# AI4Science-WestlakeU/wdno

Hardware: AMD Instinct MI355X
Metric: diffusion train steps/sec, 2D smoke U-Net (8 samples per GPU per step) (higher is better)
Workload: dtype f32

## Files before the change

### wdno_amd/csrc/conv_prep.hip

```cpp
#include "conv_tiles.h"
#include <algorithm>

template <bool RECORD>
__global__ __launch_bounds__(256) void amax_kernel(const float* __restrict__ x, int64_t n, unsigned* __restrict__ out) {
  __shared__ float red[4];
  const int64_t n4 = n >> 2;
  const float4* x4 = reinterpret_cast<const float4*>(x);
  float m = 0.f;
  const int64_t stride = (int64_t)gridDim.x * 1024;
  for (int64_t k0 = (int64_t)blockIdx.x * 1024 + threadIdx.x; k0 < n4; k0 += stride) {
    float4 v[4];
#pragma unroll
    for (int u = 0; u < 4; ++u) {
      int64_t k = k0 + u * 256;
      v[u] = k < n4 ? x4[k] : make_float4(0.f, 0.f, 0.f, 0.f);
    }
#pragma unroll
    for (int u = 0; u < 4; ++u)
      m = fmaxf(fmaxf(m, fmaxf(fabsf(v[u].x), fabsf(v[u].y))), fmaxf(fabsf(v[u].z), fabsf(v[u].w)));
  }
  if (blockIdx.x == 0)
    for (int64_t k = (n4 << 2) + threadIdx.x; k < n; k += 256) m = fmaxf(m, fabsf(x[k]));
  if (RECORD) {
    amax_record_emit(m, reinterpret_cast<float*>(out), blockIdx.x);
    return;
  }
  m = wave_max(m);
  if ((threadIdx.x & 63) == 0) red[threadIdx.x >> 6] = m;
  __syncthreads();
  if (threadIdx.x == 0) {
    m = fmaxf(fmaxf(red[0], red[1]), fmaxf(red[2], red[3]));
    atomicMax(out, __float_as_uint(m));
  }
}
void conv_amax_record_launch(const float* x, int64_t n, float* rec, hipStream_t st) {
  amax_kernel<true><<<stream_grid(n / 16 + 1, 256), 256, 0, st>>>(x, n, reinterpret_cast<unsigned*>(rec));
}
extern "C" int wdno_amax_record(const float* x, int64_t n, float* rec_zeroed, wdno_stream_t s) {
  WDNO_REQUIRE(n >= 0);
  if (n == 0) return WDNO_OK;
  amax_kernel<true><<<stream_grid(n / 16 + 1, 256), 256, 0, as_stream(s)>>>(x, n, reinterpret_cast<unsigned*>(rec_zeroed));
  return wdno_check_launch();
}
extern "C" int wdno_amax(const float* x, int64_t n, float* amax_zeroed, wdno_stream_t s) {
  WDNO_REQUIRE(n > 0);
  amax_kernel<false><<<stream_grid(n / 16 + 1, 256), 256, 0, as_stream(s)>>>(x, n, reinterpret_cast<unsigned*>(amax_zeroed));
  return wdno_check_launch();
}

__global__ __launch_bounds__(256) void split_kernel(const float* __restrict__ x, const float* __restrict__ amax,
                                                     _Float16* __restrict__ hi, _Float16* __restrict__ lo, float* __restrict__ scale_out,
                                                     int64_t rows, int C, int C8) {
  const bool lp = lo == nullptr;
  const float s = lp ? 1.0f : scale_from_amax(amax_record_read(amax));
  if (!lp && blockIdx.x == 0 && threadIdx.x == 0) scale_out[0] = s;
  const int g8 = C8 >> 3;
  const int64_t total = rows * g8;
  const int64_t stride = (int64_t)gridDim.x * 256;
  for (int64_t i = (int64_t)blockIdx.x * 256 + threadIdx.x; i < total; i += stride) {
    int64_t r = i / g8;
    int c0 = (int)(i - r * g8) * 8;
    float v[8];
    const float* xp = x + r * C + c0;
    if (c0 + 8 <= C) {
      float4 a = *reinterpret_cast<const float4*>(xp), b = *reinterpret_cast<const float4*>(xp + 4);
      v[0] = a.x; v[1] = a.y; v[2] = a.z; v[3] = a.w; v[4] = b.x; v[5] = b.y; v[6] = b.z; v[7] = b.w;
    } else {
#pragma unroll
      for (int e = 0; e < 8; ++e) v[e] = (c0 + e < C) ? xp[e] : 0.f;
    }
    if (lp) {
      typedef unsigned short us8 __attribute__((ext_vector_type(8)));
      us8 b;
#pragma unroll
      for (int e = 0; e < 8; ++e) b[e] = bf16_rne(v[e]);
      *reinterpret_cast<us8*>(hi + r * C8 + c0) = b;
      continue;
    }
    half8 h, l;
#pragma unroll
    for (int e = 0; e < 8; ++e) {
      float t = v[e] * s;
      _Float16 th = (_Float16)t;
      h[e] = th;
      l[e] = (_Float16)(t - (float)th);
    }
    *reinterpret_cast<half8*>(hi + r * C8 + c0) = h;
    *reinterpret_cast<half8*>(lo + r * C8 + c0) = l;
  }
}
extern "C" int wdno_cast_bf16(const float* x, void* out, int64_t rows, int C, int C8, wdno_stream_t s) {
  WDNO_REQUIRE(rows > 0 && C > 0 && (C & 3) == 0 && (C8 & 7) == 0 && C8 >= C && C8 < C + 16);
  int64_t total = rows * (C8 / 8);
  split_kernel<<<stream_grid(total, 256), 256, 0, as_stream(s)>>>(x, nullptr, (_Float16*)out, nullptr, nullptr, rows, C, C8);
  return wdno_check_launch();
}
extern "C" int wdno_split_f16(const float* x, const float* amax, void* hi, void* lo, float* scale_out, int64_t rows, int C, int C8,
                              wdno_stream_t s) {
  WDNO_REQUIRE(rows > 0 && C > 0 && (C & 3) == 0 && (C8 & 7) == 0 && C8 >= C && C8 < C + 16);
  int64_t total = rows * (C8 / 8);
  split_kernel<<<stream_grid(total, 256), 256, 0, as_stream(s)>>>(x, amax, (_Float16*)hi, (_Float16*)lo, scale_out, rows, C, C8);
  return wdno_check_launch();
}

__global__ __launch_bounds__(256) void split_colsum_kernel(const float* __restrict__ x, const float* __restrict__ amax,
                                                            _Float16* __restrict__ hi, _Float16* __restrict__ lo, float* __restrict__ scale_out,
                                                            double* __restrict__ part, int64_t rows, int C, int C8) {
  __shared__ float red[256][9];
  const bool lp = lo == nullptr;
  const float s = lp ? 1.0f : scale_from_amax(amax_record_read(amax));
  if (!lp && blockIdx.x == 0 && threadIdx.x == 0) scale_out[0] = s;
  const int g8 = C8 >> 3;
  const int64_t total = rows * g8;
  const int64_t stride = (int64_t)gridDim.x * 256;
  float cs[8];
#pragma unroll
  for (int e = 0; e < 8; ++e) cs[e] = 0.f;
  for (int64_t i = (int64_t)blockIdx.x * 256 + threadIdx.x; i < total; i += stride) {
    int64_t r = i / g8;
    int c0 = (int)(i - r * g8) * 8;
    float v[8];
    const float* xp = x + r * C + c0;
    if (c0 + 8 <= C) {
      float4 a = *reinterpret_cast<const float4*>(xp), b = *reinterpret_cast<const float4*>(xp + 4);
      v[0] = a.x; v[1] = a.y; v[2] = a.z; v[3] = a.w; v[4] = b.x; v[5] = b.y; v[6] = b.z; v[7] = b.w;
    } else {
#pragma unroll
      for (int e = 0; e < 8; ++e) v[e] = (c0 + e < C) ? xp[e] : 0.f;
    }
    if (lp) {
      typedef unsigned short us8 __attribute__((ext_vector_type(8)));
      us8 b;
#pragma unroll
      for (int e = 0; e < 8; ++e) { cs[e] += v[e]; b[e] = bf16_rne(v[e]); }
      *reinterpret_cast<us8*>(hi + r * C8 + c0) = b;
      continue;
    }
    half8 h, l;
#pragma unroll
    for (int e = 0; e < 8; ++e) {
      cs[e] += v[e];
      float t = v[e] * s;
      _Float16 th = (_Float16)t;
      h[e] = th;
      l[e] = (_Float16)(t - (float)th);
    }
    *reinterpret_cast<half8*>(hi + r * C8 + c0) = h;
    *reinterpret_cast<half8*>(lo + r * C8 + c0) = l;
  }
#pragma unroll
  for (int e = 0; e < 8; ++e) red[threadIdx.x][e] = cs[e];
  __syncthreads();
  for (int idx = threadIdx.x; idx < C8; idx += 256) {
    const int grp = idx >> 3, e = idx & 7;
    double acc = 0.0;
    for (int t = grp; t < 256; t += g8) acc += (double)red[t][e];
    part[(int64_t)blockIdx.x * C8 + idx] = acc;
  }
}
extern "C" size_t wdno_split_colsum_ws_bytes(int64_t rows, int C8) {
  return (size_t)stream_grid(rows * (C8 / 8), 256) * (size_t)C8 * sizeof(double);
}
extern "C" int wdno_split_f16_colsum(const float* x, const float* amax, void* hi, void* lo, float* scale_out, float* colsum_out,
                                     void* ws, size_t ws_bytes, int64_t rows, int C, int C8, wdno_stream_t s) {
  WDNO_REQUIRE(rows > 0 && C > 0 && (C & 3) == 0 && (C8 & 7) == 0 && C8 >= C && C8 < C + 16);
  const int g8 = C8 / 8;
  if (g8 > 256 || (g8 & (g8 - 1))) return WDNO_EUNSUPPORTED;
  if (ws_bytes < wdno_split_colsum_ws_bytes(rows, C8)) return WDNO_EWORKSPACE;
  const int grid = stream_grid(rows * g8, 256);
  split_colsum_kernel<<<grid, 256, 0, as_stream(s)>>>(x, amax, (_Float16*)hi, (_Float16*)lo, scale_out, (double*)ws, rows, C, C8);
  if (colsum_out)
    partial_rows_sum_kernel<double><<<cdiv(C8, 32), PRS_THREADS, 0, as_stream(s)>>>((const double*)ws, colsum_out, grid, C8);
  return wdno_check_launch();
}

extern "C" int wdno_cast_bf16_colsum(const float* x, void* out, float* colsum_out, void* ws, size_t ws_bytes, int64_t rows, int C, int C8,
                                     wdno_stream_t s) {
  WDNO_REQUIRE(rows > 0 && C > 0 && (C & 3) == 0 && (C8 & 7) == 0 && C8 >= C && C8 < C + 16);
  const int g8 = C8 / 8;
  if (g8 > 256 || (g8 & (g8 - 1))) return WDNO_EUNSUPPORTED;
  if (ws_bytes < wdno_split_colsum_ws_bytes(rows, C8)) return WDNO_EWORKSPACE;
  const int grid = stream_grid(rows * g8, 256);
  split_colsum_kernel<<<grid, 256, 0, as_stream(s)>>>(x, nullptr, (_Float16*)out, nullptr, nullptr, (double*)ws, rows, C, C8);
  if (colsum_out)
    partial_rows_sum_kernel<double><<<cdiv(C8, 32), PRS_THREADS, 0, as_stream(s)>>>((const double*)ws, colsum_out, grid, C8);
  return wdno_check_launch();
}

#define PS_LDS_FLOATS 10240
struct PackTile { int KT, CT, CTp, tiles_k, tiles_c; };
__host__ __device__ static inline PackTile pack_tile(int T, int A, int B, int mode) {
  PackTile t;
  auto need = [&](int longd, int shortd) { return (int64_t)T * (mode ? (int64_t)longd * (shortd + 1) : (int64_t)shortd * (longd + 1)); };
  int longd = 128, shortd = 8;
  while (longd > 8 && need(longd, shortd) > PS_LDS_FLOATS) longd >>= 1;
  while (shortd > 1 && need(longd, shortd) > PS_LDS_FLOATS) shortd >>= 1;
  t.KT = mode ? longd : shortd;
  t.CT = mode ? shortd : longd;
  t.CTp = t.CT + 1;
  const int kext = mode ? B : A, cext = mode ? A : B;
  t.tiles_k = (kext + t.KT - 1) / t.KT;
  t.tiles_c = (cext + t.CT - 1) / t.CT;
  return t;
}
__device__ __forceinline__ unsigned ps_magic(unsigned d) { return d > 1 ? (unsigned)((1ull << 32) / d) + 1u : 0u; }
__device__ __forceinline__ int ps_div(int n, int d, unsigned m) { return d == 1 ? n : (int)__umulhi((unsigned)n, m); }
__device__ __forceinline__ void pack_split_body(const float* __restrict__ w, const float* __restrict__ amax,
                                                _Float16* __restrict__ hi, _Float16* __restrict__ lo,
                                                float* __restrict__ scale_out, int K, int C, int kd, int kh, int kw,
                                                int A, int B, int mode_in, int block, int nblocks) {
  __shared__ float tile[PS_LDS_FLOATS + 16];
  const int frag = mode_in >= 10 ? mode_in - 9 : 0;
  const int parity = mode_in >= 2 && mode_in < 6 ? mode_in - 2 : -1;
  const int patch = mode_in >= 6 && mode_in < 10 ? mode_in - 6 : -1;
  const int mode = mode_in == 1 || patch >= 0 ? 1 : 0;
  const bool lp = lo == nullptr;
  const float s = lp ? 1.0f : scale_from_amax(amax[0]);
  if (!lp && block == 0 && threadIdx.x == 0) scale_out[0] = s;
  const int b8 = B >> 3;
  const int T = kd * kh * kw, khw = kh * kw;
  const PackTile pt = pack_tile(T, A, B, mode);
  if ((int64_t)T * pt.KT * pt.CTp > PS_LDS_FLOATS + 16) return;
  const int ntiles = pt.tiles_k * pt.tiles_c;
  const int run = pt.CT * T;
  const int bt8 = (mode ? pt.KT : pt.CT) >> 3;
  const int at = mode ? pt.CT : pt.KT;
  const unsigned m_run = ps_magic(run), m_T = ps_magic(T), m_bt8 = ps_magic(bt8), m_at = ps_magic(at), m_khw = ps_magic(khw), m_kw = ps_magic(kw);
  for (int tl = block; tl < ntiles; tl += nblocks) {
    const int tk = ps_div(tl, pt.tiles_c, ps_magic(pt.tiles_c)), tc = tl - tk * pt.tiles_c;
    const int k0 = tk * pt.KT, c0 = tc * pt.CT;
    __syncthreads();
    const int cvalid = min(pt.CT, C - c0);
    const int nload = pt.KT * run;
    for (int idx0 = threadIdx.x; idx0 < nload; idx0 += 256 * 8) {
      float v[8];
      int dst[8];
#pragma unroll
      for (int u = 0; u < 8; ++u) {
        const int idx = min(idx0 + 256 * u, nload - 1);
        const int kk = ps_div(idx, run, m_run), r = idx - kk * run;
        const int cl = ps_div(r, T, m_T), tap = r - cl * T;
        const bool ok = k0 + kk < K && cl < cvalid;
        const int64_t off = !ok ? 0 : patch >= 0 ? (((int64_t)(k0 + kk) * C + c0 + cl) * 4 + patch) : parity < 0 ? ((int64_t)(k0 + kk) * C + c0) * T + r
                            : ((int64_t)(c0 + cl) * K + (k0 + kk)) * 16 + (3 - (parity >> 1) - 2 * (tap >> 1)) * 4 + (3 - (parity & 1) - 2 * (tap & 1));
        v[u] = w[off];
        if (!ok) v[u] = 0.f;
        dst[u] = idx0 + 256 * u < nload ? (tap * pt.KT + kk) * pt.CTp + cl : -1;
      }
#pragma unroll
      for (int u = 0; u < 8; ++u)
        if (dst[u] >= 0) tile[dst[u]] = v[u];
    }
    __syncthreads();
    const int nitems = T * at * bt8;
    for (int idx = threadIdx.x; idx < nitems; idx += 256) {
      int q = ps_div(idx, bt8, m_bt8);
      const int g = idx - q * bt8;
      const int tap = ps_div(q, at, m_at), al = q - tap * at;
      const int dz = ps_div(tap, khw, m_khw), rr = tap - dz * khw;
      const int dy = ps_div(rr, kw, m_kw), dx = rr - dy * kw;
      const int ts = mode ? T - 1 - tap : tap;
      const int a = (mode ? c0 : k0) + al;
      const int bg = ((mode ? k0 : c0) >> 3) + g;
      if (a >= A || bg >= b8) continue;
      const float* src = mode ? tile + (ts * pt.KT + g * 8) * pt.CTp + al : tile + (ts * pt.KT + al) * pt.CTp + g * 8;
      const int step = mode ? pt.CTp : 1;
      half8 h, l;
      typedef unsigned short us8 __attribute__((ext_vector_type(8)));
      us8 bq;
#pragma unroll
      for (int e = 0; e < 8; ++e) {
        const float v = src[e * step];
        const float tv = v * s;
        const _Float16 th = (_Float16)tv;
        h[e] = th;
        l[e] = (_Float16)(tv - (float)th);
        bq[e] = bf16_rne(v);
      }
      int64_t i = ((((int64_t)dz * kh + dy) * A + a) * kw + dx) * b8 + bg;
      if (frag) {
        const int li = a & 31, t = bg >> 2, hh2 = (bg >> 1) & 1, s2 = bg & 1;
        if (frag == 1) { const int ti = a >> 7, hd = (a >> 5) & 3; i = ((((hd * 3 + ti) * (B >> 5) + t) * 2 + s2) * 64 + hh2 * 32 + li); }
        else { const int q4 = A >> 2, wv = a / q4, mt = (a - wv * q4) >> 5; i = ((((wv * (A >> 7) + mt) * 4 + t) * 2 + s2) * 64 + hh2 * 32 + li); }
      }
      if (lp) { *reinterpret_cast<us8*>(hi + i * 8) = bq; continue; }
      *reinterpret_cast<half8*>(hi + i * 8) = h;
      *reinterpret_cast<half8*>(lo + i * 8) = l;
    }
  }
}
__global__ __launch_bounds__(256) void pack_split_weight_kernel(const float* __restrict__ w, const float* __restrict__ amax,
                                                                 _Float16* __restrict__ hi, _Float16* __restrict__ lo,
                                                                 float* __restrict__ scale_out, int K, int C, int kd, int kh, int kw,
                                                                 int A, int B, int mode) {
  pack_split_body(w, amax, hi, lo, scale_out, K, C, kd, kh, kw, A, B, mode, (int)blockIdx.x, (int)gridDim.x);
}
__global__ __launch_bounds__(256) void amax_multi_kernel(const wdno_amax_item* __restrict__ tab) {
  __shared__ float red[4];
  const wdno_amax_item it = tab[blockIdx.y];
  const float* x = (const float*)it.x;
  const int64_t n = it.n;
  float m = 0.f;
  int64_t head = (int64_t)(((16 - (reinterpret_cast<uintptr_t>(x) & 15)) & 15) >> 2);
  if (head > n) head = n;
  const int64_t n4 = (n - head) >> 2, tail0 = head + 4 * n4;
  if (blockIdx.x == 0) {
    if ((int64_t)threadIdx.x < head) m = fabsf(x[threadIdx.x]);
    if (tail0 + (int64_t)threadIdx.x < n) m = fmaxf(m, fabsf(x[tail0 + threadIdx.x]));
  }
  const float4* x4 = reinterpret_cast<const float4*>(x + head);
  const int64_t stride = (int64_t)gridDim.x * 256;
  int64_t k = (int64_t)blockIdx.x * 256 + threadIdx.x;
  for (; k + 3 * stride < n4; k += 4 * stride) {
    const float4 a = x4[k], b = x4[k + stride], c = x4[k + 2 * stride], d = x4[k + 3 * stride];
    m = amax4(amax4(m, a), b);
    m = amax4(amax4(m, c), d);
  }
  for (; k < n4; k += stride) m = amax4(m, x4[k]);
  m = wave_max(m);
  if ((threadIdx.x & 63) == 0) red[threadIdx.x >> 6] = m;
  __syncthreads();
  if (threadIdx.x == 0) {
    m = fmaxf(fmaxf(red[0], red[1]), fmaxf(red[2], red[3]));
    if (m > 0.f) atomicMax((unsigned*)it.out, __float_as_uint(m));
  }
}
extern "C" int wdno_amax_multi(const void* table, int n_items, int blocks_per_item, wdno_stream_t s) {
  WDNO_REQUIRE(table && n_items > 0 && n_items <= 65535 && blocks_per_item > 0);
  amax_multi_kernel<<<dim3((unsigned)blocks_per_item, (unsigned)n_items), 256, 0, as_stream(s)>>>((const wdno_amax_item*)table);
  return wdno_check_launch();
}
__global__ __launch_bounds__(256) void pack_split_weight_multi_kernel(const wdno_wsplit_item* __restrict__ tab) {
  const wdno_wsplit_item it = tab[blockIdx.y];
  pack_split_body((const float*)it.w, (const float*)it.amax, (_Float16*)it.hi, (_Float16*)it.lo, (float*)it.scale_out, it.K, it.C, it.kd, it.kh,
                  it.kw, it.A, it.B, it.mode, (int)blockIdx.x, (int)gridDim.x);
}
extern "C" int wdno_pack_split_weight_multi(const void* table, int n_items, int blocks_per_item, wdno_stream_t s) {
  WDNO_REQUIRE(table && n_items > 0 && n_items <= 65535 && blocks_per_item > 0);
  pack_split_weight_multi_kernel<<<dim3((unsigned)blocks_per_item, (unsigned)n_items), 256, 0, as_stream(s)>>>((const wdno_wsplit_item*)table);
  return wdno_check_launch();
}
extern "C" int wdno_pack_split_weight(const float* w, const float* amax, void* hi, void* lo, float* scale_out, int K, int C, int kd, int kh,
                                      int kw, int A, int B, int mode, wdno_stream_t s) {
  WDNO_REQUIRE(K > 0 && C > 0 && kd > 0 && kh > 0 && kw > 0 && A > 0 && B > 0 && (B & 7) == 0 && mode >= 0 && mode <= 11);
  WDNO_REQUIRE(mode < 2 || mode > 5 || (kd == 1 && kh == 2 && kw == 2));
  WDNO_REQUIRE(mode < 6 || (kd == 1 && kh == 1 && kw == 1));
  WDNO_REQUIRE(mode != 1 && (mode < 6 || mode >= 10) ? (A >= K && B >= C) : (A >= C && B >= K));
  WDNO_REQUIRE(mode != 10 || (A == 384 && (B & 31) == 0 && lo != nullptr));
  WDNO_REQUIRE(mode != 11 || (B == 128 && (A & 127) == 0 && lo != nullptr));
  WDNO_REQUIRE(lo == nullptr || (amax != nullptr && scale_out != nullptr));
  int64_t total = (int64_t)kd * kh * A * kw * (B / 8);
  const PackTile ptile = pack_tile(kd * kh * kw, A, B, mode == 1 || (mode >= 6 && mode < 10) ? 1 : 0);
  if ((int64_t)kd * kh * kw * ptile.KT * ptile.CTp > PS_LDS_FLOATS + 16) return WDNO_EUNSUPPORTED;
  (void)total;
  pack_split_weight_kernel<<<std::min(2048, ptile.tiles_k * ptile.tiles_c), 256, 0, as_stream(s)>>>(w, amax, (_Float16*)hi, (_Float16*)lo, scale_out, K, C, kd, kh, kw,
                                                                            A, B, mode);
  return wdno_check_launch();
}
```

### wdno_amd/csrc/conv_wgrad_h3.hip

```cpp
#include "conv_tiles.h"

__device__ __forceinline__ __amdgpu_buffer_rsrc_t make_rsrc(const void* ptr, unsigned bytes) {
  return __builtin_amdgcn_make_buffer_rsrc(const_cast<void*>(ptr), (short)0, (int)bytes, 0x00020000);
}

typedef _Float16 half4 __attribute__((ext_vector_type(4)));
#define WH_BKP 32
#define WH_PAD 32

__global__ __launch_bounds__(256) void pixel_table_kernel(int4v* __restrict__ tbl, wdno_conv_geom g, int P) {
  int p = blockIdx.x * 256 + threadIdx.x;
  if (p >= P) return;
  int q = p;
  int ow = q % g.OW; q /= g.OW;
  int oh = q % g.OH; q /= g.OH;
  int od = q % g.OD;
  int n = q / g.OD;
  int d0 = od * g.sd - g.pd, h0 = oh * g.sh - g.ph, w0 = ow * g.sw - g.pw;
  int4v e;
  e.x = ((n * g.YD + (od * g.osd + g.ood)) * g.YH + (oh * g.osh + g.ooh)) * g.YW + (ow * g.osw + g.oow);
  e.y = (((n * g.D + d0) * g.H + h0) * g.W + w0) * g.C;
  e.z = (d0 << 16) | (h0 & 0xffff);
  e.w = w0;
  tbl[p] = e;
}
extern "C" int wdno_conv_pixel_table(void* table, const wdno_conv_geom* g, wdno_stream_t s) {
  int rc = check_geom(g);
  if (rc) return rc;
  int64_t P = (int64_t)g->N * g->OD * g->OH * g->OW;
  if (P >= 0x7fffffff || (int64_t)g->N * g->D * g->H * g->W * g->C >= 0x3fffffff) return WDNO_EUNSUPPORTED;
  pixel_table_kernel<<<(unsigned)cdiv64(P, 256), 256, 0, as_stream(s)>>>((int4v*)table, *g, (int)P);
  return wdno_check_launch();
}

struct WgradHP {
  ConvP c;
  int tiles_k, tiles_r, splits, bn;
  int64_t pix_per_split;
  int xcd_group;
};

__device__ __forceinline__ half8 tr_frag(const _Float16* tile, int stride, int pix0, int ch0, int lane) {
  const int g = lane >> 4, xl = lane & 15;
  const _Float16* p0 = tile + (pix0 + 8 * (g >> 1) + (xl >> 2)) * stride + ch0 + 16 * (g & 1) + 4 * (xl & 3);
  typedef short short4v __attribute__((ext_vector_type(4)));
  typedef short4v __attribute__((address_space(3))) * lds_s4;
  short4v a = __builtin_amdgcn_ds_read_tr16_b64_v4i16((lds_s4)(p0));
  short4v b = __builtin_amdgcn_ds_read_tr16_b64_v4i16((lds_s4)(p0 + 4 * stride));
  typedef short short8v __attribute__((ext_vector_type(8)));
  short8v c = __builtin_shufflevector(a, b, 0, 1, 2, 3, 4, 5, 6, 7);
  return __builtin_bit_cast(half8, c);
}

#define WH_RING 4
template <int BM, int BN, int WM, int WN, bool LP>
__global__ __launch_bounds__(256) void conv_wgrad_h3_kernel(const _Float16* __restrict__ xh, const _Float16* __restrict__ xl,
                                                             const _Float16* __restrict__ dyh, const _Float16* __restrict__ dyl,
                                                             const float* __restrict__ sx, const float* __restrict__ sdy,
                                                             const int4v* __restrict__ table, float* __restrict__ ws, WgradHP wpz,
                                                             unsigned x_bytes, unsigned dy_bytes) {
  constexpr int TM = BM / (WM * 32);
  constexpr int TN = BN / (WN * 32);
  constexpr int SA = BM + WH_PAD, SB = BN + WH_PAD;
  constexpr int A_C8 = BM / 8, B_C8 = BN / 8;
  constexpr int A_RPP = 256 / A_C8;
  constexpr int A_PASSES = WH_BKP / A_RPP, B_PASSES = WH_BKP * B_C8 / 256;
  static_assert(256 % A_C8 == 0 && (WH_BKP * B_C8) % 256 == 0, "loader mapping");
  constexpr int NPL = LP ? 1 : 2;
  constexpr int STAGE = NPL * WH_BKP * (SA + SB);
  extern __shared__ __attribute__((aligned(16))) _Float16 hsm[];
  int4v* pinfo = reinterpret_cast<int4v*>(hsm + 2 * STAGE);

  const ConvP& p = wpz.c;
  const wdno_conv_geom& g = p.g;
  const int tid = threadIdx.x;
  int b = wpz.xcd_group ? xcd_swizzle((int)(blockIdx.y * gridDim.x + blockIdx.x), (int)(gridDim.x * gridDim.y))
                        : (int)(blockIdx.y * gridDim.x + blockIdx.x);
  const int split = b / (int)gridDim.x;
  b -= split * (int)gridDim.x;
  const int tile_r = b % wpz.tiles_r; b /= wpz.tiles_r;
  const int tap = b % (g.kd * g.kh);
  const int tile_k = b / (g.kd * g.kh);
  const int dz = tap / g.kh, dyy = tap - dz * g.kh;
  const int k0 = tile_k * BM, r0 = tile_r * BN;
  const int pbeg = (int)((int64_t)split * wpz.pix_per_split);
  int pend = pbeg + (int)wpz.pix_per_split;
  if (pend > (int)p.P) pend = (int)p.P;
  const int nsteps = pbeg < pend ? (pend - pbeg + WH_BKP - 1) / WH_BKP : 0;
  const __amdgpu_buffer_rsrc_t rxh = make_rsrc(xh, x_bytes), rxl = make_rsrc(xl, x_bytes);
  const __amdgpu_buffer_rsrc_t rdh = make_rsrc(dyh, dy_bytes), rdl = make_rsrc(dyl, dy_bytes);
  const int tap_off = (dz * g.H + dyy) * g.W * g.C;

  auto fetch_rec = [&](int step) -> int4v {
    int4v e;
    e.x = 0; e.y = 0; e.z = (int)0x80008000; e.w = 0;
    int pm = pbeg + step * WH_BKP + tid;
    if (tid < WH_BKP && step < nsteps && pm < pend) e = table[pm];
    if (tid < WH_BKP && !(step < nsteps && pm < pend)) e.x = -1;
    return e;
  };
  auto put_rec = [&](int step, int4v e) {
    if (tid < WH_BKP) pinfo[(step & (WH_RING - 1)) * WH_BKP + tid] = e;
  };

  int b_row[B_PASSES], b_c8[B_PASSES], r[B_PASSES], dx[B_PASSES];
  bool r_ok[B_PASSES];
#pragma unroll
  for (int i = 0; i < B_PASSES; ++i) {
    const int idx = tid + 256 * i;
    b_row[i] = idx / B_C8;
    b_c8[i] = (idx - b_row[i] * B_C8) * 8;
    r[i] = r0 + b_c8[i];
    r_ok[i] = r[i] < p.R;
    dx[i] = r[i] / g.C;
  }
  const int a_row = tid / A_C8, a_c8 = (tid % A_C8) * 8;
  const int ka = k0 + a_c8;
  const bool ka_ok = ka < g.K;

  int4v ah[A_PASSES], al[A_PASSES], bh[B_PASSES], bl[B_PASSES];
  auto load_tile = [&](int step) {
    const int4v* ps = pinfo + (step & (WH_RING - 1)) * WH_BKP;
#pragma unroll
    for (int i = 0; i < A_PASSES; ++i) {
      const int4v e = ps[a_row + i * A_RPP];
      const int off = (e.x >= 0 && ka_ok) ? (e.x * g.K + ka) * 2 : CV_OOB;
      ah[i] = __builtin_amdgcn_raw_buffer_load_b128(rdh, off, 0, 0);
      if (!LP) al[i] = __builtin_amdgcn_raw_buffer_load_b128(rdl, off, 0, 0);
    }
#pragma unroll
    for (int i = 0; i < B_PASSES; ++i) {
      const int4v e = ps[b_row[i]];
      const int d = (e.z >> 16) + dz, h = (int)(short)(e.z & 0xffff) + dyy, w = e.w + dx[i];
      const bool ok = e.x >= 0 && r_ok[i] && (unsigned)d < (unsigned)g.D && (unsigned)h < (unsigned)g.H && (unsigned)w < (unsigned)g.W;
      const int off = ok ? (e.y + tap_off + r[i]) * 2 : CV_OOB;
      bh[i] = __builtin_amdgcn_raw_buffer_load_b128(rxh, off, 0, 0);
      if (!LP) bl[i] = __builtin_amdgcn_raw_buffer_load_b128(rxl, off, 0, 0);
    }
  };
  auto store_tile = [&](int buf) {
    _Float16* Ah = hsm + buf * STAGE;
    _Float16* Al = Ah + WH_BKP * SA;
    _Float16* Bh = Ah + NPL * WH_BKP * SA;
    _Float16* Bl = Bh + WH_BKP * SB;
#pragma unroll
    for (int i = 0; i < A_PASSES; ++i) {
      *reinterpret_cast<int4v*>(&Ah[(a_row + i * A_RPP) * SA + a_c8]) = ah[i];
      if (!LP) *reinterpret_cast<int4v*>(&Al[(a_row + i * A_RPP) * SA + a_c8]) = al[i];
    }
#pragma unroll
    for (int i = 0; i < B_PASSES; ++i) {
      *reinterpret_cast<int4v*>(&Bh[b_row[i] * SB + b_c8[i]]) = bh[i];
      if (!LP) *reinterpret_cast<int4v*>(&Bl[b_row[i] * SB + b_c8[i]]) = bl[i];
// ... 172 lines not shown
  }
  size_t need = (size_t)w.splits * g->kd * g->kh * (size_t)g->K * w.c.R * sizeof(float);
  float* wsf = (w.splits == 1 && single) ? single : (float*)ws;
  if (wsf == (float*)ws && ws_bytes < need) return WDNO_EWORKSPACE;
  if (w.splits > 65535) return WDNO_EUNSUPPORTED;
  dim3 grid((unsigned)(w.tiles_k * g->kd * g->kh * w.tiles_r), (unsigned)w.splits);
  if (xl == nullptr) {
    if (pl.bm == 128) launch_wgrad_h3<128, 192, 2, 2, true>(xh, xh, dyh, dyh, sx, sdy, pixel_table, wsf, w, grid, st);
    else if (w.bn == 192) launch_wgrad_h3<64, 192, 2, 2, true>(xh, xh, dyh, dyh, sx, sdy, pixel_table, wsf, w, grid, st);
    else launch_wgrad_h3<64, 128, 1, 4, true>(xh, xh, dyh, dyh, sx, sdy, pixel_table, wsf, w, grid, st);
  } else if (pl.bm == 128) launch_wgrad_h3<128, 192, 2, 2, false>(xh, xl, dyh, dyl, sx, sdy, pixel_table, wsf, w, grid, st);
  else if (w.bn == 192) launch_wgrad_h3<64, 192, 2, 2, false>(xh, xl, dyh, dyl, sx, sdy, pixel_table, wsf, w, grid, st);
  else launch_wgrad_h3<64, 128, 1, 4, false>(xh, xl, dyh, dyl, sx, sdy, pixel_table, wsf, w, grid, st);
  *splits_out = w.splits;
  return WDNO_OK;
}
extern "C" int wdno_conv_wgrad_f16x3(const void* xh, const void* xl, const float* sx, const void* dyh, const void* dyl, const float* sdy,
                                     const void* pixel_table, float* dwp, void* ws, size_t ws_bytes, const wdno_conv_geom* g, wdno_stream_t s) {
  hipStream_t st = as_stream(s);
  int splits = 0;
  int rc = wgrad_h3_partials(xh, xl, sx, dyh, dyl, sdy, pixel_table, dwp, ws, ws_bytes, g, st, &splits);
  if (rc) return rc;
  if (splits > 1) {
    int64_t n = (int64_t)g->kd * g->kh * g->K * (int64_t)g->kw * g->C;
    wgrad_h3_reduce_kernel<<<stream_grid(n / 4 + 1, 256), 256, 0, st>>>((const float*)ws, dwp, n, splits);
  }
  return wdno_check_launch();
}
__device__ __forceinline__ void wgrad_h3_reduce_nat_body(const float* __restrict__ ws, float* __restrict__ dw, int64_t n, int splits,
                                                         int K8, int C8, int kw, int ntap, int Kn, int Cn, float4 (*part)[33], int bid, int nb) {
  const int R = kw * C8;
  const int j = threadIdx.x & 31, q = threadIdx.x >> 5;
  const int64_t n4 = n >> 2;
  for (int64_t i4 = (int64_t)bid * 32 + j; i4 - j < n4; i4 += (int64_t)nb * 32) {
    float4 a = make_float4(0.f, 0.f, 0.f, 0.f), b = a;
    if (i4 < n4) {
      const float4* src = reinterpret_cast<const float4*>(ws) + i4;
      int sidx = q;
      for (; sidx + 8 < splits; sidx += 16) {
        const float4 u = src[(int64_t)sidx * n4], v = src[(int64_t)(sidx + 8) * n4];
        a.x += u.x; a.y += u.y; a.z += u.z; a.w += u.w;
        b.x += v.x; b.y += v.y; b.z += v.z; b.w += v.w;
      }
      if (sidx < splits) {
        const float4 u = src[(int64_t)sidx * n4];
        a.x += u.x; a.y += u.y; a.z += u.z; a.w += u.w;
      }
    }
    part[q][j] = make_float4(a.x + b.x, a.y + b.y, a.z + b.z, a.w + b.w);
    __syncthreads();
    if (q < 4 && i4 < n4) {
      float t = 0.f;
#pragma unroll
      for (int g = 0; g < 8; ++g) {
        const float4 v = part[g][j];
        t += q == 0 ? v.x : q == 1 ? v.y : q == 2 ? v.z : v.w;
      }
      const int64_t i = i4 * 4 + q;
      const int r = (int)(i % R);
      int64_t tt = i / R;
      const int k = (int)(tt % K8);
      const int tap = (int)(tt / K8);
      const int dx = r / C8, c = r - dx * C8;
      if (k < Kn && c < Cn) dw[(((int64_t)k * Cn + c) * ntap + tap) * kw + dx] = t;
    }
    __syncthreads();
  }
}
__global__ __launch_bounds__(256) void wgrad_h3_reduce_nat_kernel(const float* __restrict__ ws, float* __restrict__ dw, int64_t n, int splits,
                                                                   int K8, int C8, int kw, int ntap, int Kn, int Cn) {
  __shared__ float4 part[8][33];
  wgrad_h3_reduce_nat_body(ws, dw, n, splits, K8, C8, kw, ntap, Kn, Cn, part, (int)blockIdx.x, (int)gridDim.x);
}
__device__ __forceinline__ void wgrad_h3_reduce_tile_body(const float* __restrict__ ws, float* __restrict__ dw, int64_t n, int splits,
                                                          int K8, int C8, int kw, int ntap, int Kn, int Cn, float (*tile)[65], int bx, int by) {
  const int T = ntap * kw, R = kw * C8;
  const int k = by, c0 = bx * 64;
  const int wave = threadIdx.x >> 6, lane = threadIdx.x & 63;
  for (int sgm = wave; sgm < T; sgm += 4) {
    const int t = sgm / kw, dx = sgm - t * kw;
    float a = 0.f, b = 0.f;
    if (c0 + lane < C8) {
      const float* src = ws + ((int64_t)t * K8 + k) * R + dx * C8 + c0 + lane;
      int sp = 0;
      for (; sp + 1 < splits; sp += 2) { a += src[(int64_t)sp * n]; b += src[(int64_t)(sp + 1) * n]; }
      if (sp < splits) a += src[(int64_t)sp * n];
    }
    tile[lane][sgm] = a + b;
  }
  __syncthreads();
  const int cn = min(64, Cn - c0);
  float* out = dw + ((int64_t)k * Cn + c0) * T;
  for (int e = threadIdx.x; e < cn * T; e += 256) {
    const int c = e / T, sgm = e - c * T;
    out[e] = tile[c][sgm];
  }
}
__global__ __launch_bounds__(256) void wgrad_h3_reduce_tile_kernel(const float* __restrict__ ws, float* __restrict__ dw, int64_t n, int splits,
                                                                    int K8, int C8, int kw, int ntap, int Kn, int Cn) {
  __shared__ float tile[64][65];
  wgrad_h3_reduce_tile_body(ws, dw, n, splits, K8, C8, kw, ntap, Kn, Cn, tile, (int)blockIdx.x, (int)blockIdx.y);
}
static bool wgrad_h3_reduce_tiled(int splits, const wdno_conv_geom* g, int Kn, int Cn) {
  const int T = g->kd * g->kh * g->kw;
  const bool big = (int64_t)Kn * cdiv(Cn, 64) >= 512 && splits <= 8;
  return T <= 64 && (splits <= 2 || big);
}
extern "C" int wdno_conv_wgrad_plan(const wdno_conv_geom* g, int lowp, int Kn, int Cn, wdno_wgrad_plan* out) {
  (void)lowp;
  WDNO_REQUIRE(out);
  int rc = check_geom(g);
  if (rc) return rc;
  if ((g->C & 7) || (g->K & 7)) return WDNO_EUNSUPPORTED;
  WgradHP w;
  rc = wgrad_h3_choose(g, w, *out);
  if (rc) return rc;
  out->reduce_tiled = wgrad_h3_reduce_tiled(out->splits, g, Kn > 0 ? Kn : g->K, Cn > 0 ? Cn : g->C) ? 1 : 0;
  return WDNO_OK;
}

struct WgradReduceArgs {
  wdno_wgrad_reduce_item it[WDNO_WGRAD_REDUCE_MAX];
  int first[WDNO_WGRAD_REDUCE_MAX + 1];
  int n;
};
__global__ __launch_bounds__(256) void wgrad_h3_reduce_multi_kernel(const WgradReduceArgs a) {
  __shared__ __attribute__((aligned(16))) float smem[64 * 65];
  int lo = 0, hi = a.n - 1;
  while (lo < hi) {
    const int mid = (lo + hi + 1) >> 1;
    if (a.first[mid] <= (int)blockIdx.x) lo = mid; else hi = mid - 1;
  }
  const wdno_wgrad_reduce_item& w = a.it[lo];
  const int bid = (int)blockIdx.x - a.first[lo], nb = a.first[lo + 1] - a.first[lo];
  if (w.tiled) {
    const int bxn = (w.Cn + 63) >> 6;
    wgrad_h3_reduce_tile_body(w.ws, w.dw, w.n, w.splits, w.K8, w.C8, w.kw, w.ntap, w.Kn, w.Cn, reinterpret_cast<float (*)[65]>(smem), bid % bxn, bid / bxn);
  } else {
    wgrad_h3_reduce_nat_body(w.ws, w.dw, w.n, w.splits, w.K8, w.C8, w.kw, w.ntap, w.Kn, w.Cn, reinterpret_cast<float4 (*)[33]>(smem), bid, nb);
  }
}
extern "C" int wdno_wgrad_reduce_multi(const wdno_wgrad_reduce_item* items, int n_items, wdno_stream_t s) {
  WDNO_REQUIRE(items && n_items >= 0);
  hipStream_t st = as_stream(s);
  for (int base = 0; base < n_items; base += WDNO_WGRAD_REDUCE_MAX) {
    WgradReduceArgs a;
    a.n = n_items - base < WDNO_WGRAD_REDUCE_MAX ? n_items - base : WDNO_WGRAD_REDUCE_MAX;
    int grid = 0;
    for (int i = 0; i < a.n; ++i) {
      a.it[i] = items[base + i];
      const wdno_wgrad_reduce_item& w = a.it[i];
      WDNO_REQUIRE(w.ws && w.dw && w.n > 0 && w.splits >= 1 && w.Kn > 0 && w.Cn > 0 && w.Kn <= w.K8 && w.Cn <= w.C8);
      a.first[i] = grid;
      grid += w.tiled ? cdiv(w.Cn, 64) * w.Kn : stream_grid(w.n / 4, 32);
    }
    a.first[a.n] = grid;
    if (grid > 0) wgrad_h3_reduce_multi_kernel<<<grid, 256, 0, st>>>(a);
  }
  return wdno_check_launch();
}

static void wgrad_h3_reduce_launch(const float* ws, float* dw, int64_t n, int splits, const wdno_conv_geom* g, int Kn, int Cn, hipStream_t st) {
  if (wgrad_h3_reduce_tiled(splits, g, Kn, Cn)) {
    wgrad_h3_reduce_tile_kernel<<<dim3(cdiv(Cn, 64), Kn), 256, 0, st>>>(ws, dw, n, splits, g->K, g->C, g->kw, g->kd * g->kh, Kn, Cn);
    return;
  }
  wgrad_h3_reduce_nat_kernel<<<stream_grid(n / 4, 32), 256, 0, st>>>(ws, dw, n, splits, g->K, g->C, g->kw, g->kd * g->kh, Kn, Cn);
}
extern "C" int wdno_conv_wgrad_f16x3_param(const void* xh, const void* xl, const float* sx, const void* dyh, const void* dyl, const float* sdy,
                                           const void* pixel_table, float* dw, int Kn, int Cn, void* ws, size_t ws_bytes,
                                           const wdno_conv_geom* g, wdno_stream_t s) {
  WDNO_REQUIRE(g && Kn > 0 && Cn > 0 && Kn <= g->K && Cn <= g->C);
  hipStream_t st = as_stream(s);
  int splits = 0;
  int rc = wgrad_h3_partials(xh, xl, sx, dyh, dyl, sdy, pixel_table, nullptr, ws, ws_bytes, g, st, &splits);
  if (rc) return rc;
  const int64_t n = (int64_t)g->kd * g->kh * g->K * (int64_t)g->kw * g->C;
  wgrad_h3_reduce_launch((const float*)ws, dw, n, splits, g, Kn, Cn, st);
  return wdno_check_launch();
}

extern "C" int wdno_conv_wgrad_partials(const void* xh, const void* xl, const float* sx, const void* dyh, const void* dyl, const float* sdy,
                                        const void* pixel_table, float* dw, int Kn, int Cn, void* ws, size_t ws_bytes,
                                        const wdno_conv_geom* g, wdno_wgrad_reduce_item* item, wdno_stream_t s) {
  WDNO_REQUIRE(g && item && dw && Kn > 0 && Cn > 0 && Kn <= g->K && Cn <= g->C);
  int splits = 0;
  int rc = wgrad_h3_partials(xh, xl, sx, dyh, dyl, sdy, pixel_table, nullptr, ws, ws_bytes, g, as_stream(s), &splits);
  if (rc) return rc;
  const int64_t n = (int64_t)g->kd * g->kh * g->K * (int64_t)g->kw * g->C;
  if (n >= 0x7fffffff) return WDNO_EUNSUPPORTED;
  item->ws = (const float*)ws; item->dw = dw; item->n = (int)n; item->splits = splits; item->K8 = g->K; item->C8 = g->C; item->kw = g->kw;
  item->ntap = g->kd * g->kh; item->Kn = Kn; item->Cn = Cn; item->tiled = wgrad_h3_reduce_tiled(splits, g, Kn, Cn) ? 1 : 0;
  return wdno_check_launch();
}

extern "C" int wdno_conv_wgrad_bf16_param(const void* x16, const void* dy16, const void* pixel_table, float* dw, int Kn, int Cn, void* ws,
                                          size_t ws_bytes, const wdno_conv_geom* g, wdno_stream_t s) {
  WDNO_REQUIRE(g && Kn > 0 && Cn > 0 && Kn <= g->K && Cn <= g->C);
  hipStream_t st = as_stream(s);
  int splits = 0;
  int rc = wgrad_h3_partials(x16, nullptr, nullptr, dy16, nullptr, nullptr, pixel_table, nullptr, ws, ws_bytes, g, st, &splits);
  if (rc) return rc;
  const int64_t n = (int64_t)g->kd * g->kh * g->K * (int64_t)g->kw * g->C;
  wgrad_h3_reduce_launch((const float*)ws, dw, n, splits, g, Kn, Cn, st);
  return wdno_check_launch();
}
```

Before: 32.62.

## Vectorize weight pack loads, flatten multi-item pack into pooled tile scheduling

The weight split/pack kernel is rewritten to process one tile per call. It uses float4 row loads with alignment handling for the plain layout, a padded LDS pitch that allows float4 reads, and shift-based index decoding. The multi-item pack kernel now runs on a flat pool of blocks that load-balance over tiles using a block prefix scan and a binary search, replacing the fixed 2D grid. The wgrad reduce grid size is factored into a shared helper. The aim is to cut uncoalesced scalar loads and idle blocks in the per-step weight preprocessing. The cost is extra complexity and some per-block scan overhead.

```diff
diff --git a/wdno_amd/csrc/conv_prep.hip b/wdno_amd/csrc/conv_prep.hip
--- a/wdno_amd/csrc/conv_prep.hip
+++ b/wdno_amd/csrc/conv_prep.hip
@@ -1,4 +1,5 @@
 #include "conv_tiles.h"
+#include "weight_path.h"
 #include <algorithm>
 
 template <bool RECORD>
@@ -187,51 +188,85 @@
   return wdno_check_launch();
 }
 
-#define PS_LDS_FLOATS 10240
-struct PackTile { int KT, CT, CTp, tiles_k, tiles_c; };
-__host__ __device__ static inline PackTile pack_tile(int T, int A, int B, int mode) {
-  PackTile t;
-  auto need = [&](int longd, int shortd) { return (int64_t)T * (mode ? (int64_t)longd * (shortd + 1) : (int64_t)shortd * (longd + 1)); };
-  int longd = 128, shortd = 8;
-  while (longd > 8 && need(longd, shortd) > PS_LDS_FLOATS) longd >>= 1;
-  while (shortd > 1 && need(longd, shortd) > PS_LDS_FLOATS) shortd >>= 1;
-  t.KT = mode ? longd : shortd;
-  t.CT = mode ? shortd : longd;
-  t.CTp = t.CT + 1;
-  const int kext = mode ? B : A, cext = mode ? A : B;
-  t.tiles_k = (kext + t.KT - 1) / t.KT;
-  t.tiles_c = (cext + t.CT - 1) / t.CT;
-  return t;
-}
-__device__ __forceinline__ unsigned ps_magic(unsigned d) { return d > 1 ? (unsigned)((1ull << 32) / d) + 1u : 0u; }
+__device__ __forceinline__ unsigned ps_magic(unsigned d) { return d > 1 ? 0xffffffffu / d + 1u : 0u; }
 __device__ __forceinline__ int ps_div(int n, int d, unsigned m) { return d == 1 ? n : (int)__umulhi((unsigned)n, m); }
-__device__ __forceinline__ void pack_split_body(const float* __restrict__ w, const float* __restrict__ amax,
+__device__ __forceinline__ int ps_log2(int p) { return 31 - __clz(p); }
+#define PS_INFLIGHT 10
+__device__ __forceinline__ void pack_split_tile(const float* __restrict__ w, const float* __restrict__ amax,
                                                 _Float16* __restrict__ hi, _Float16* __restrict__ lo,
                                                 float* __restrict__ scale_out, int K, int C, int kd, int kh, int kw,
-                                                int A, int B, int mode_in, int block, int nblocks) {
-  __shared__ float tile[PS_LDS_FLOATS + 16];
+                                                int A, int B, int mode_in, int tl, float* __restrict__ tile) {
   const int frag = mode_in >= 10 ? mode_in - 9 : 0;
   const int parity = mode_in >= 2 && mode_in < 6 ? mode_in - 2 : -1;
   const int patch = mode_in >= 6 && mode_in < 10 ? mode_in - 6 : -1;
-  const int mode = mode_in == 1 || patch >= 0 ? 1 : 0;
+  const int mode = wp_pack_dgrad(mode_in);
   const bool lp = lo == nullptr;
-  const float s = lp ? 1.0f : scale_from_amax(amax[0]);
-  if (!lp && block == 0 && threadIdx.x == 0) scale_out[0] = s;
+  const float am = lp ? 0.f : amax[0];
   const int b8 = B >> 3;
-  const int T = kd * kh * kw, khw = kh * kw;
+  const int T = kd * kh * kw;
   const PackTile pt = pack_tile(T, A, B, mode);
-  if ((int64_t)T * pt.KT * pt.CTp > PS_LDS_FLOATS + 16) return;
-  const int ntiles = pt.tiles_k * pt.tiles_c;
+  const int L = mode ? pt.KT : pt.CT, S = mode ? pt.CT : pt.KT;
+  const int Lp = wp_pack_pitch(T, S, L);
+  const int st = S * Lp;
+  const int sk = mode ? 1 : Lp, sc = mode ? Lp : 1;
   const int run = pt.CT * T;
-  const int bt8 = (mode ? pt.KT : pt.CT) >> 3;
-  const int at = mode ? pt.CT : pt.KT;
-  const unsigned m_run = ps_magic(run), m_T = ps_magic(T), m_bt8 = ps_magic(bt8), m_at = ps_magic(at), m_khw = ps_magic(khw), m_kw = ps_magic(kw);
-  for (int tl = block; tl < ntiles; tl += nblocks) {
-    const int tk = ps_div(tl, pt.tiles_c, ps_magic(pt.tiles_c)), tc = tl - tk * pt.tiles_c;
-    const int k0 = tk * pt.KT, c0 = tc * pt.CT;
-    __syncthreads();
-    const int cvalid = min(pt.CT, C - c0);
+  const int tk = tl / pt.tiles_c, tc = tl - tk * pt.tiles_c;
+  const int k0 = tk * pt.KT, c0 = tc * pt.CT;
+  const int cvalid = max(0, min(pt.CT, C - c0));
+  const unsigned m_T = ps_magic(T), m_kw = ps_magic(kw);
+  __syncthreads();
+  if (parity < 0 && patch < 0) {
+    const int len = cvalid * T;
+    const int npc = (run + 6) >> 2;
+    const unsigned m_npc = ps_magic(npc);
+    const int aw = (int)((reinterpret_cast<uintptr_t>(w) >> 2) & 3);
+    const int npieces = pt.KT * npc;
+    for (int idx0 = threadIdx.x; idx0 < npieces; idx0 += 256 * PS_INFLIGHT) {
+      float4 v[PS_INFLIGHT];
+      int r0[PS_INFLIGHT], kks[PS_INFLIGHT];
+#pragma unroll
+      for (int u = 0; u < PS_INFLIGHT; ++u) {
+        r0[u] = run;
+        kks[u] = 0;
+        if (idx0 - (int)threadIdx.x + 256 * u >= npieces) continue;
+        const int idx = idx0 + 256 * u;
+        const int kk = ps_div(min(idx, npieces - 1), npc, m_npc), j = idx - kk * npc;
+        const int64_t rowoff = ((int64_t)(k0 + kk) * C + c0) * T;
+        const int a = (aw + (int)(rowoff & 3)) & 3;
+        const int r = 4 * j - a;
+        const int rowlen = idx < npieces && k0 + kk < K ? len : 0;
+        const float* p = w + rowoff + r;
+        v[u] = make_float4(0.f, 0.f, 0.f, 0.f);
+        if (r >= 0 && r + 4 <= rowlen) v[u] = *reinterpret_cast<const float4*>(p);
+        else if (r + 4 > 0 && r < rowlen) {
+          if (r >= 0) v[u].x = p[0];
+          if (r + 1 >= 0 && r + 1 < rowlen) v[u].y = p[1];
+          if (r + 2 >= 0 && r + 2 < rowlen) v[u].z = p[2];
+          if (r + 3 < rowlen) v[u].w = p[3];
+        }
+        if (idx < npieces) r0[u] = r;
+        kks[u] = kk;
+      }
+#pragma unroll
+      for (int u = 0; u < PS_INFLIGHT; ++u) {
+        if (idx0 - (int)threadIdx.x + 256 * u >= npieces) continue;
+        const int rs = max(r0[u], 0);
+        int cl = ps_div(rs, T, m_T), tap = rs - cl * T;
+        float* dst = tile + kks[u] * sk;
+        const float e[4] = {v[u].x, v[u].y, v[u].z, v[u].w};
+#pragma unroll
+        for (int q = 0; q < 4; ++q) {
+          const int r = r0[u] + q;
+          if (r >= 0 && r < run) {
+            dst[tap * st + cl * sc] = e[q];
+            if (++tap == T) { tap = 0; ++cl; }
+          }
+        }
+      }
+    }
+  } else {
     const int nload = pt.KT * run;
+    const unsigned m_run = ps_magic(run);
     for (int idx0 = threadIdx.x; idx0 < nload; idx0 += 256 * 8) {
       float v[8];
       int dst[8];
@@ -241,59 +276,90 @@
         const int kk = ps_div(idx, run, m_run), r = idx - kk * run;
         const int cl = ps_div(r, T, m_T), tap = r - cl * T;
         const bool ok = k0 + kk < K && cl < cvalid;
-        const int64_t off = !ok ? 0 : patch >= 0 ? (((int64_t)(k0 + kk) * C + c0 + cl) * 4 + patch) : parity < 0 ? ((int64_t)(k0 + kk) * C + c0) * T + r
+        const int64_t off = !ok ? 0 : patch >= 0 ? (((int64_t)(k0 + kk) * C + c0 + cl) * 4 + patch)
                             : ((int64_t)(c0 + cl) * K + (k0 + kk)) * 16 + (3 - (parity >> 1) - 2 * (tap >> 1)) * 4 + (3 - (parity & 1) - 2 * (tap & 1));
         v[u] = w[off];
         if (!ok) v[u] = 0.f;
-        dst[u] = idx0 + 256 * u < nload ? (tap * pt.KT + kk) * pt.CTp + cl : -1;
+        dst[u] = idx0 + 256 * u < nload ? tap * st + kk * sk + cl * sc : -1;
       }
 #pragma unroll
       for (int u = 0; u < 8; ++u)
         if (dst[u] >= 0) tile[dst[u]] = v[u];
     }
-    __syncthreads();
-    const int nitems = T * at * bt8;
-    for (int idx = threadIdx.x; idx < nitems; idx += 256) {
-      int q = ps_div(idx, bt8, m_bt8);
-      const int g = idx - q * bt8;
-      const int tap = ps_div(q, at, m_at), al = q - tap * at;
-      const int dz = ps_div(tap, khw, m_khw), rr = tap - dz * khw;
-      const int dy = ps_div(rr, kw, m_kw), dx = rr - dy * kw;
-      const int ts = mode ? T - 1 - tap : tap;
-      const int a = (mode ? c0 : k0) + al;
-      const int bg = ((mode ? k0 : c0) >> 3) + g;
-      if (a >= A || bg >= b8) continue;
-      const float* src = mode ? tile + (ts * pt.KT + g * 8) * pt.CTp + al : tile + (ts * pt.KT + al) * pt.CTp + g * 8;
-      const int step = mode ? pt.CTp : 1;
-      half8 h, l;
+  }
+  __syncthreads();
+  const float s = lp ? 1.0f : scale_from_amax(am);
+  if (!lp && tl == 0 && threadIdx.x == 0) scale_out[0] = s;
+  const int lb = ps_log2(L >> 3), ls = ps_log2(S);
+  const int nitems = (T * S) << lb;
+  const bool wide = (Lp & 3) == 0;
+  for (int idx = threadIdx.x; idx < nitems; idx += 256) {
+    const int g = idx & ((1 << lb) - 1), q = idx >> lb;
+    const int al = q & (S - 1), tap = q >> ls;
+    const int th = ps_div(tap, kw, m_kw), dx = tap - th * kw;
+    const int ts = mode ? T - 1 - tap : tap;
+    const int a = (mode ? c0 : k0) + al;
+    const int bg = ((mode ? k0 : c0) >> 3) + g;
+    if (a >= A || bg >= b8) continue;
+    const float* src = tile + ts * st + al * Lp + g * 8;
+    float v[8];
+    if (wide) {
+      const float4 x = *reinterpret_cast<const float4*>(src), y = *reinterpret_cast<const float4*>(src + 4);
+      v[0] = x.x; v[1] = x.y; v[2] = x.z; v[3] = x.w; v[4] = y.x; v[5] = y.y; v[6] = y.z; v[7] = y.w;
+    } else {
+#pragma unroll
+      for (int e = 0; e < 8; ++e) v[e] = src[e];
+    }
+    int64_t i = (((int64_t)th * A + a) * kw + dx) * b8 + bg;
+    if (frag) {
+      const int li = a & 31, t = bg >> 2, hh2 = (bg >> 1) & 1, s2 = bg & 1;
+      if (frag == 1) { const int ti = a >> 7, hd = (a >> 5) & 3; i = ((((hd * 3 + ti) * (B >> 5) + t) * 2 + s2) * 64 + hh2 * 32 + li); }
+      else { const int q4 = A >> 2, wv = a / q4, mt = (a - wv * q4) >> 5; i = ((((wv * (A >> 7) + mt) * 4 + t) * 2 + s2) * 64 + hh2 * 32 + li); }
+    }
+    if (lp) {
       typedef unsigned short us8 __attribute__((ext_vector_type(8)));
       us8 bq;
 #pragma unroll
-      for (int e = 0; e < 8; ++e) {
-        const float v = src[e * step];
-        const float tv = v * s;
-        const _Float16 th = (_Float16)tv;
-        h[e] = th;
-        l[e] = (_Float16)(tv - (float)th);
-        bq[e] = bf16_rne(v);
-      }
-      int64_t i = ((((int64_t)dz * kh + dy) * A + a) * kw + dx) * b8 + bg;
-      if (frag) {
-        const int li = a & 31, t = bg >> 2, hh2 = (bg >> 1) & 1, s2 = bg & 1;
-        if (frag == 1) { const int ti = a >> 7, hd = (a >> 5) & 3; i = ((((hd * 3 + ti) * (B >> 5) + t) * 2 + s2) * 64 + hh2 * 32 + li); }
-        else { const int q4 = A >> 2, wv = a / q4, mt = (a - wv * q4) >> 5; i = ((((wv * (A >> 7) + mt) * 4 + t) * 2 + s2) * 64 + hh2 * 32 + li); }
-      }
-      if (lp) { *reinterpret_cast<us8*>(hi + i * 8) = bq; continue; }
-      *reinterpret_cast<half8*>(hi + i * 8) = h;
-      *reinterpret_cast<half8*>(lo + i * 8) = l;
-    }
+      for (int e = 0; e < 8; ++e) bq[e] = bf16_rne(v[e]);
+      *reinterpret_cast<us8*>(hi + i * 8) = bq;
+      continue;
+    }
+    half8 h, l;
+#pragma unroll
+    for (int e = 0; e < 8; ++e) {
+      const float tv = v[e] * s;
+      const _Float16 th16 = (_Float16)tv;
+      h[e] = th16;
+      l[e] = (_Float16)(tv - (float)th16);
+    }
+    *reinterpret_cast<half8*>(hi + i * 8) = h;
+    *reinterpret_cast<half8*>(lo + i * 8) = l;
   }
 }
 __global__ __launch_bounds__(256) void pack_split_weight_kernel(const float* __restrict__ w, const float* __restrict__ amax,
                                                                  _Float16* __restrict__ hi, _Float16* __restrict__ lo,
                                                                  float* __restrict__ scale_out, int K, int C, int kd, int kh, int kw,
                                                                  int A, int B, int mode) {
-  pack_split_body(w, amax, hi, lo, scale_out, K, C, kd, kh, kw, A, B, mode, (int)blockIdx.x, (int)gridDim.x);
+  __shared__ __attribute__((aligned(16))) float tile[PS_LDS_FLOATS + 16];
+  const int ntiles = wp_pack_tiles(kd * kh * kw, A, B, mode);
+  for (int tl = (int)blockIdx.x; tl < ntiles; tl += (int)gridDim.x)
+    pack_split_tile(w, amax, hi, lo, scale_out, K, C, kd, kh, kw, A, B, mode, tl, tile);
+}
+#define WP_POOL_BLOCKS 2048
+__device__ __forceinline__ void wp_block_scan(int cnt, int* first, int* wsum) {
+  const int lane = threadIdx.x & 63, wave = threadIdx.x >> 6;
+  int v = cnt;
+#pragma unroll
+  for (int o = 1; o < 64; o <<= 1) {
+    const int u = __shfl_up(v, o, 64);
+    if (lane >= o) v += u;
+  }
+  if (lane == 63) wsum[wave] = v;
+  __syncthreads();
+  for (int w = 0; w < wave; ++w) v += wsum[w];
+  first[threadIdx.x + 1] = v;
+  if (threadIdx.x == 0) first[0] = 0;
+  __syncthreads();
 }
 __global__ __launch_bounds__(256) void amax_multi_kernel(const wdno_amax_item* __restrict__ tab) {
   __shared__ float red[4];
@@ -330,14 +396,36 @@
   amax_multi_kernel<<<dim3((unsigned)blocks_per_item, (unsigned)n_items), 256, 0, as_stream(s)>>>((const wdno_amax_item*)table);
   return wdno_check_launch();
 }
-__global__ __launch_bounds__(256) void pack_split_weight_multi_kernel(const wdno_wsplit_item* __restrict__ tab) {
-  const wdno_wsplit_item it = tab[blockIdx.y];
-  pack_split_body((const float*)it.w, (const float*)it.amax, (_Float16*)it.hi, (_Float16*)it.lo, (float*)it.scale_out, it.K, it.C, it.kd, it.kh,
-                  it.kw, it.A, it.B, it.mode, (int)blockIdx.x, (int)gridDim.x);
+__global__ __launch_bounds__(256) void pack_split_weight_multi_kernel(const wdno_wsplit_item* __restrict__ tab, int n_items) {
+  __shared__ __attribute__((aligned(16))) float tile[PS_LDS_FLOATS + 16];
+  __shared__ int first[257], wsum[4];
+  const int G = (int)gridDim.x;
+  int rot = 0;
+  for (int ib = 0; ib < n_items; ib += 256) {
+    const int ni = min(256, n_items - ib);
+    int cnt = 0;
+    if ((int)threadIdx.x < ni) {
+      const wdno_wsplit_item& it = tab[ib + threadIdx.x];
+      cnt = wp_pack_tiles(it.kd * it.kh * it.kw, it.A, it.B, it.mode);
+    }
+    __syncthreads();
+    wp_block_scan(cnt, first, wsum);
+    const int total = first[ni];
+    int cur = -1;
+    wdno_wsplit_item it;
+    for (int f = wp_first_unit((int)blockIdx.x, G, rot); f < total; f += G) {
+      const int i = __builtin_amdgcn_readfirstlane(wp_find_item(first, ni, f));
+      if (i != cur) { it = tab[ib + i]; cur = i; }
+      pack_split_tile((const float*)it.w, (const float*)it.amax, (_Float16*)it.hi, (_Float16*)it.lo, (float*)it.scale_out, it.K, it.C, it.kd, it.kh,
+                      it.kw, it.A, it.B, it.mode, f - first[i], tile);
+    }
+    rot = (rot + total % G) % G;
+  }
 }
 extern "C" int wdno_pack_split_weight_multi(const void* table, int n_items, int blocks_per_item, wdno_stream_t s) {
   WDNO_REQUIRE(table && n_items > 0 && n_items <= 65535 && blocks_per_item > 0);
-  pack_split_weight_multi_kernel<<<dim3((unsigned)blocks_per_item, (unsigned)n_items), 256, 0, as_stream(s)>>>((const wdno_wsplit_item*)table);
+  const int grid = (int)std::min<int64_t>((int64_t)blocks_per_item * n_items, WP_POOL_BLOCKS);
+  pack_split_weight_multi_kernel<<<grid, 256, 0, as_stream(s)>>>((const wdno_wsplit_item*)table, n_items);
   return wdno_check_launch();
 }
 extern "C" int wdno_pack_split_weight(const float* w, const float* amax, void* hi, void* lo, float* scale_out, int K, int C, int kd, int kh,
diff --git a/wdno_amd/csrc/conv_wgrad_h3.hip b/wdno_amd/csrc/conv_wgrad_h3.hip
--- a/wdno_amd/csrc/conv_wgrad_h3.hip
+++ b/wdno_amd/csrc/conv_wgrad_h3.hip
@@ -1,4 +1,5 @@
 #include "conv_tiles.h"
+#include "weight_path.h"
 
 __device__ __forceinline__ __amdgpu_buffer_rsrc_t make_rsrc(const void* ptr, unsigned bytes) {
   return __builtin_amdgcn_make_buffer_rsrc(const_cast<void*>(ptr), (short)0, (int)bytes, 0x00020000);
@@ -477,7 +478,7 @@
       const wdno_wgrad_reduce_item& w = a.it[i];
       WDNO_REQUIRE(w.ws && w.dw && w.n > 0 && w.splits >= 1 && w.Kn > 0 && w.Cn > 0 && w.Kn <= w.K8 && w.Cn <= w.C8);
       a.first[i] = grid;
-      grid += w.tiled ? cdiv(w.Cn, 64) * w.Kn : stream_grid(w.n / 4, 32);
+      grid += wp_reduce_blocks(w.tiled, w.n, w.Kn, w.Cn);
     }
     a.first[a.n] = grid;
     if (grid > 0) wgrad_h3_reduce_multi_kernel<<<grid, 256, 0, st>>>(a);
@@ -490,7 +491,7 @@
     wgrad_h3_reduce_tile_kernel<<<dim3(cdiv(Cn, 64), Kn), 256, 0, st>>>(ws, dw, n, splits, g->K, g->C, g->kw, g->kd * g->kh, Kn, Cn);
     return;
   }
-  wgrad_h3_reduce_nat_kernel<<<stream_grid(n / 4, 32), 256, 0, st>>>(ws, dw, n, splits, g->K, g->C, g->kw, g->kd * g->kh, Kn, Cn);
+  wgrad_h3_reduce_nat_kernel<<<wp_reduce_blocks(0, n, Kn, Cn), 256, 0, st>>>(ws, dw, n, splits, g->K, g->C, g->kw, g->kd * g->kh, Kn, Cn);
 }
 extern "C" int wdno_conv_wgrad_f16x3_param(const void* xh, const void* xl, const float* sx, const void* dyh, const void* dyl, const float* sdy,
                                            const void* pixel_table, float* dw, int Kn, int Cn, void* ws, size_t ws_bytes,
diff --git a/wdno_amd/csrc/weight_path.h b/wdno_amd/csrc/weight_path.h
--- /dev/null
+++ b/wdno_amd/csrc/weight_path.h
@@ -0,0 +1,47 @@
+#pragma once
+#include <stdint.h>
+#if defined(__HIPCC__)
+#define WP_HD __host__ __device__
+#else
+#define WP_HD
+#endif
+
+#define PS_LDS_FLOATS 10240
+struct PackTile { int KT, CT, CTp, tiles_k, tiles_c; };
+WP_HD static inline PackTile pack_tile(int T, int A, int B, int mode) {
+  PackTile t;
+  auto need = [&](int longd, int shortd) { return (int64_t)T * (mode ? (int64_t)longd * (shortd + 1) : (int64_t)shortd * (longd + 1)); };
+  int longd = 128, shortd = 8;
+  while (longd > 8 && need(longd, shortd) > PS_LDS_FLOATS) longd >>= 1;
+  while (shortd > 1 && need(longd, shortd) > PS_LDS_FLOATS) shortd >>= 1;
+  t.KT = mode ? longd : shortd;
+  t.CT = mode ? shortd : longd;
+  t.CTp = t.CT + 1;
+  const int kext = mode ? B : A, cext = mode ? A : B;
+  t.tiles_k = (kext + t.KT - 1) / t.KT;
+  t.tiles_c = (cext + t.CT - 1) / t.CT;
+  return t;
+}
+WP_HD static inline int wp_pack_dgrad(int mode_in) { return mode_in == 1 || (mode_in >= 6 && mode_in < 10) ? 1 : 0; }
+WP_HD static inline int wp_pack_pitch(int T, int S, int L) { return (int64_t)T * S * (L + 4) <= PS_LDS_FLOATS + 16 ? L + 4 : L + 1; }
+WP_HD static inline int wp_pack_tiles(int T, int A, int B, int mode_in) {
+  const PackTile pt = pack_tile(T, A, B, wp_pack_dgrad(mode_in));
+  if ((int64_t)T * pt.KT * pt.CTp > PS_LDS_FLOATS + 16) return 0;
+  return pt.tiles_k * pt.tiles_c;
+}
+
+WP_HD static inline int wp_reduce_blocks(int tiled, int64_t n, int Kn, int Cn) {
+  if (tiled) return ((Cn + 63) / 64) * Kn;
+  const int64_t g = (n / 4 + 31) / 32;
+  return g > 2048 ? 2048 : g < 1 ? 1 : (int)g;
+}
+
+WP_HD static inline int wp_find_item(const int* first, int n, int f) {
+  int lo = 0, hi = n - 1;
+  while (lo < hi) {
+    const int mid = (lo + hi + 1) >> 1;
+    if (first[mid] <= f) lo = mid; else hi = mid - 1;
+  }
+  return lo;
+}
+WP_HD static inline int wp_first_unit(int b, int G, int rot) { return ((b - rot) % G + G) % G; }
```

Result: no change. 32.72 (median of 6 runs) (+0.3%).
